# shayekh00/Knowledge_Distillation_for_Sensory_Substitution_in_Multimodal_Models

Hardware: AMD Instinct MI355X
Metric: KD samples/sec/step (7B->0.5B, 336x336) (higher is better)
Workload: dtype bf16; 1 GPU; c1: logit-based KD (LoCa, T=1), 7B->0.5B, 336x336; model=llava-onevision-qwen2-7b (teacher) -> 0.5b (student), global_batch=4, per_gpu_batch=4, seq_len=1536, image=336x336 (2 tiles, 1485 tokens), parallelism=dp1, teacher_lm_stream=bf16

## Files before the change

### knowledge_distillation_for_sensory_substitution_in_multimodal_models_amd/csrc/gemm.hip

```cpp
#include "common.h"

#include <cstring>
#include <type_traits>
#ifdef KD_AB_BUILD
#include <hipblaslt/hipblaslt.h>
#endif

namespace kd {
namespace {

constexpr int BM = 128, BN = 128, BK = 64, NTH = 256;
constexpr int TILE_BYTES = 128 * 64 * 2;
constexpr uint32_t OOB = 0x80000000u;

typedef __attribute__((address_space(3))) void lds_void_t;
typedef __attribute__((address_space(3))) bf16x4 lds_bf16x4_t;

struct GemmP {
    const bf16* A; const bf16* B; void* C;
    const void* bias; const bf16* resid; bf16* aux; const float* alpha_dev;
    int64_t lda, ldb, ldc, ldr, ld_aux;
    int M, N, K;
    float alpha;
    int c_f32, accumulate, bias_f32, act, res_mod;
    int res_f32;
    bf16 *sq, *sk, *sv;
    const float *rcos, *rsin;
    int sS, snq, snkv, shd, shdp;
    int64_t kchunk;
    int64_t split_stride;
    int glu;
    int tile0;
    const float* sa;
    const float* sb;
    int gx, gy;
    float* rst;
    int rst_nt, rst_vs, rst_top2;
    float rst_inv_t;
    int sk_steps, sk_grid;
    float* sk_ws;
    int sk_dp;
    int* sk_cnt;
    int gm;
    int stagger;
    int stag_g;
};

__host__ __device__ inline int sk_wg_of(int64_t s, int64_t tot, int G) { return (int)(((s + 1) * G - 1) / tot); }

__device__ __forceinline__ uint32_t sw_k(int row) { return (uint32_t)((row >> 1) & 7); }
__device__ __forceinline__ uint32_t sw_mn(int k) { return (uint32_t)(((k & 3) | (((k >> 3) & 1) << 2)) << 1); }

__device__ __forceinline__ uint32_t rec_bytes(int64_t rows, int64_t ld) {
    const int64_t b = rows * ld * 2;
    return b <= 0 ? 0u : (b >= 0x7FFFFFFFll ? 0x7FFFFFFFu : (uint32_t)b);
}

__device__ __forceinline__ __amdgpu_buffer_rsrc_t make_rsrc(const void* base, uint32_t bytes) {
    return __builtin_amdgcn_make_buffer_rsrc(const_cast<void*>(base), (short)0, (int)bytes, 0x00020000);
}

__device__ __forceinline__ void dma16(__amdgpu_buffer_rsrc_t rs, char* lds_dst, uint32_t voff) {
    __builtin_amdgcn_raw_ptr_buffer_load_lds(rs, (lds_void_t*)lds_dst, 16, voff, 0, 0, 0);
}

template <bool MN>
__device__ __forceinline__ void stage(char* tile, const bf16* ptr, int64_t ld, int r0, int rows_total,
                                      int k0, int K, int wid, int lane) {
    if (!MN) {
        const int rows_valid = min(128, rows_total - r0);
        auto rs = make_rsrc(ptr + (int64_t)r0 * ld, rec_bytes(rows_valid, ld));
#pragma unroll
        for (int s = 0; s < 4; ++s) {
            const int i = wid * 4 + s;
            const int row = 8 * i + (lane >> 3);
            const int gc = (lane & 7) ^ (int)sw_k(row);
            const int k = k0 + gc * 8;
            const uint32_t voff = (k < K) ? (uint32_t)(((int64_t)row * ld + k) * 2) : OOB;
            dma16(rs, tile + i * 1024, voff);
        }
    } else {
        const int kvalid = max(0, min(64, K - k0));
        auto rs = make_rsrc(ptr + (int64_t)min(k0, K) * ld + r0, rec_bytes(kvalid, ld));
#pragma unroll
        for (int s = 0; s < 4; ++s) {
            const int i = wid * 4 + s;
            const int kr = 4 * i + (lane >> 4);
            const int gc = (lane & 15) ^ (int)sw_mn(kr);
            const int row = r0 + gc * 8;
            const uint32_t voff = (kr < kvalid && row < rows_total) ? (uint32_t)(((int64_t)kr * ld + gc * 8) * 2) : OOB;
            dma16(rs, tile + i * 1024, voff);
        }
    }
}

template <bool MN>
__device__ __forceinline__ bf16x8 frag(const char* tile, int rb, int ks, int lane) {
    if (!MN) {
        const int r = rb + (lane & 15);
        const int kc = ks * 4 + (lane >> 4);
        return *(const bf16x8*)(tile + r * 128 + ((kc ^ (int)sw_k(r)) << 4));
    } else {
        const int g = lane >> 4, q = (lane & 15) >> 2, p = lane & 3;
        const int cc = (rb >> 3) + (p >> 1);
        const int kr0 = ks * 32 + 8 * g + q;
        const int kr1 = kr0 + 4;
        const char* a0 = tile + kr0 * 256 + ((cc ^ (int)sw_mn(kr0)) << 4) + ((p & 1) << 3);
        const char* a1 = tile + kr1 * 256 + ((cc ^ (int)sw_mn(kr1)) << 4) + ((p & 1) << 3);
        bf16x4 h0 = __builtin_amdgcn_ds_read_tr16_b64_v4bf16((lds_bf16x4_t*)a0);
        bf16x4 h1 = __builtin_amdgcn_ds_read_tr16_b64_v4bf16((lds_bf16x4_t*)a1);
        bf16x8 r;
        r[0] = h0[0]; r[1] = h0[1]; r[2] = h0[2]; r[3] = h0[3];
        r[4] = h1[0]; r[5] = h1[1]; r[6] = h1[2]; r[7] = h1[3];
        return r;
    }
}

__device__ __forceinline__ float gelu_tanh(float x) {
    constexpr float c0 = -2.f * 0.7978845608028654f * 1.4426950408889634f;
    constexpr float c1 = c0 * 0.044715f;
    const float e = __builtin_amdgcn_exp2f(x * fmaf(c1, x * x, c0));
    return x * __builtin_amdgcn_rcpf(1.f + e);
}
__device__ __forceinline__ float gelu_erf(float x) { return 0.5f * x * (1.f + erff(x * 0.7071067811865476f)); }
// ... 119 lines not shown
                }
            }
        }
    }
}


constexpr int EPI_G = 8, QKV_G = 2;
constexpr int BK2 = 32, NST = 4, NTH2 = 512;

__device__ __forceinline__ int f4(int row) { return (0x1320 >> (((row >> 2) & 3) * 4)) & 3; }

template <int R, bool MN>
__device__ __forceinline__ void stage2(char* tile, const bf16* ptr, int64_t ld, int r0, int rows_total, int k0, int K,
                                       int wid, int lane, __amdgpu_buffer_rsrc_t rs_k) {
    constexpr int NI = R / 16;
    constexpr int PER = NI / 8;
    if (!MN) {
#pragma unroll
        for (int s = 0; s < PER; ++s) {
            const int i = wid * PER + s;
            const int row = 16 * i + (lane >> 2);
            const int gc = (lane & 3) ^ f4(row);
            const int k = k0 + gc * 8;
            const uint32_t voff = (k < K) ? (uint32_t)(((int64_t)row * ld + k) * 2) : OOB;
            dma16(rs_k, tile + i * 1024, voff);
        }
    } else {
        constexpr int CPR = R / 8;
        constexpr int KPI = 64 / CPR;
        const int kvalid = max(0, min(BK2, K - k0));
        auto rs = make_rsrc(ptr + (int64_t)min(k0, K) * ld + r0, rec_bytes(kvalid, ld));
#pragma unroll
        for (int s = 0; s < PER; ++s) {
            const int i = wid * PER + s;
            const int kr = i * KPI + lane / CPR;
            const int gc = (lane % CPR) ^ (int)sw_mn(kr);
            const int row = r0 + gc * 8;
            const uint32_t voff = (kr < kvalid && row < rows_total) ? (uint32_t)(((int64_t)kr * ld + gc * 8) * 2) : OOB;
            dma16(rs, tile + i * 1024, voff);
        }
    }
}

template <int OFF>
__device__ __forceinline__ bf16x4 ds_read_tr_asm(const char* lds) {
    u32x2 r;
    asm volatile("ds_read_b64_tr_b16 %0, %1 offset:%2" : "=v"(r) : "v"((uint32_t)(uintptr_t)lds), "i"(OFF));
    return __builtin_bit_cast(bf16x4, r);
}

template <int R, bool MN>
__device__ __forceinline__ bf16x8 frag2(const char* tile, int rb, int lane) {
    if (!MN) {
        const int r = rb + (lane & 15);
        const int c = lane >> 4;
        return *(const bf16x8*)(tile + r * 64 + ((c ^ f4(r)) << 4));
    } else {
        constexpr int RB = R * 2;
        const int g = lane >> 4, q = (lane & 15) >> 2, p = lane & 3;
        const int cc = (rb >> 3) + (p >> 1);
        const int kr0 = 8 * g + q;
        const char* a0 = tile + kr0 * RB + ((cc ^ (int)sw_mn(kr0)) << 4) + ((p & 1) << 3);
        const bf16x4 h0 = ds_read_tr_asm<0>(a0);
        const bf16x4 h1 = ds_read_tr_asm<4 * RB>(a0);
        bf16x8 r;
        r[0] = h0[0]; r[1] = h0[1]; r[2] = h0[2]; r[3] = h0[3];
        r[4] = h1[0]; r[5] = h1[1]; r[6] = h1[2]; r[7] = h1[3];
        return r;
    }
}

template <int N> __device__ __forceinline__ void wait_vm() {
    if constexpr (N == 0) asm volatile("s_waitcnt vmcnt(0)" ::: "memory");
    else if constexpr (N == 2) asm volatile("s_waitcnt vmcnt(2)" ::: "memory");
    else if constexpr (N == 3) asm volatile("s_waitcnt vmcnt(3)" ::: "memory");
    else if constexpr (N == 4) asm volatile("s_waitcnt vmcnt(4)" ::: "memory");
    else if constexpr (N == 6) asm volatile("s_waitcnt vmcnt(6)" ::: "memory");
    else if constexpr (N == 8) asm volatile("s_waitcnt vmcnt(8)" ::: "memory");
    else if constexpr (N == 9) asm volatile("s_waitcnt vmcnt(9)" ::: "memory");
    else if constexpr (N == 12) asm volatile("s_waitcnt vmcnt(12)" ::: "memory");
    else if constexpr (N == 15) asm volatile("s_waitcnt vmcnt(15)" ::: "memory");
    else if constexpr (N == 16) asm volatile("s_waitcnt vmcnt(16)" ::: "memory");
    else if constexpr (N == 24) asm volatile("s_waitcnt vmcnt(24)" ::: "memory");
    else static_assert(N == 0, "unsupported vmcnt");
}

template <int BM, int BN, int NS = NST>
constexpr size_t gemm2_lds() {
    constexpr size_t ring = (size_t)NS * (BM + BN) * BK2 * 2;
    constexpr size_t ep16 = (size_t)BM * (BN * 2 + 16);
    constexpr size_t ep32 = (size_t)(BM / 2) * (BN * 4 + 16);
    return ring > ep16 ? (ring > ep32 ? ring : ep32) : (ep16 > ep32 ? ep16 : ep32);
}


__device__ __forceinline__ int acc_row(int lane) { return lane & 15; }
__device__ __forceinline__ int acc_col(int lane) { return (lane >> 4) * 4; }

template <bool L32>
__device__ __forceinline__ int acc_col_of(int j, int lane) {
    return L32 ? (j >> 2) * 32 + 8 * (j & 3) + 4 * (lane >> 5) : j * 16 + acc_col(lane);
}

template <int ACT, int TM, int TN, int MT, int NT, bool F32, bool L32 = false>
__device__ __forceinline__ void epi_to_lds(const f32x4 (&acc)[MT][NT], char* smem, int rs, float alpha,
                                           const f32x4 (&bcol)[NT], int wm, int wn, int lane, int r_lo, int r_hi) {
#pragma unroll
    for (int i = 0; i < MT; ++i) {
        const int lr0 = wm * TM + i * (L32 ? 32 : 16);
        if (lr0 < r_lo || lr0 >= r_hi) continue;
        const int lr = lr0 - r_lo + (L32 ? (lane & 31) : acc_row(lane));
#pragma unroll
        for (int j = 0; j < NT; ++j) {
            const f32x4 a = acc[i][j];
            const int lc = wn * TN + acc_col_of<L32>(j, lane);
            float v[4];
#pragma unroll
            for (int r = 0; r < 4; ++r) v[r] = apply_act(a[r] * alpha + bcol[j][r], ACT);
            if (F32) *(f32x4*)(smem + lr * rs + lc * 4) = (f32x4){v[0], v[1], v[2], v[3]};
            else *(bf16x4*)(smem + lr * rs + lc * 2) = (bf16x4){(bf16)v[0], (bf16)v[1], (bf16)v[2], (bf16)v[3]};
        }
    }
}

template <int TM, int TN, int MT, int NT, bool F32, bool L32 = false>
__device__ __forceinline__ void epi_to_lds_act(int act, const f32x4 (&acc)[MT][NT], char* smem, int rs, float alpha,
                                               const f32x4 (&bcol)[NT], int wm, int wn, int lane, int r_lo, int r_hi) {
    switch (act) {
        case KD_ACT_GELU_TANH: epi_to_lds<KD_ACT_GELU_TANH, TM, TN, MT, NT, F32, L32>(acc, smem, rs, alpha, bcol, wm, wn, lane, r_lo, r_hi); break;
        case KD_ACT_GELU_ERF: epi_to_lds<KD_ACT_GELU_ERF, TM, TN, MT, NT, F32, L32>(acc, smem, rs, alpha, bcol, wm, wn, lane, r_lo, r_hi); break;
        case KD_ACT_SILU: epi_to_lds<KD_ACT_SILU, TM, TN, MT, NT, F32, L32>(acc, smem, rs, alpha, bcol, wm, wn, lane, r_lo, r_hi); break;
        default: epi_to_lds<KD_ACT_NONE, TM, TN, MT, NT, F32, L32>(acc, smem, rs, alpha, bcol, wm, wn, lane, r_lo, r_hi); break;
    }
}

template <int ROWS, int BN, int NTHR, bool F32, bool RES, bool RF, bool ACC>
__device__ __forceinline__ void epi_flush_g(const GemmP& p, const char* smem, int rs, void* dst_, int64_t ld, int m0,
                                            int n0, int tid, bool full) {
    constexpr int EPC = F32 ? 4 : 8;
    constexpr int CPR = BN / EPC;
    static_assert(NTHR % CPR == 0 && (ROWS * CPR) % NTHR == 0, "epi_flush: chunk map");
    constexpr int RSTEP = NTHR / CPR, PER = ROWS * CPR / NTHR, G = PER < EPI_G ? PER : EPI_G;
    static_assert(PER % G == 0, "epi_flush: group");
    using RT = std::conditional_t<RF, f32x4, std::conditional_t<F32, bf16x4, bf16x8>>;
    using VT = std::conditional_t<F32, f32x4, bf16x8>;
    const int c = tid % CPR, lr0 = tid / CPR;
    const int col = n0 + c * EPC;
    if (!full && col >= p.N) return;
#pragma unroll 1
    for (int g0 = 0; g0 < PER; g0 += G) {
        RT rv[G];
        VT cv[G];
        if constexpr (RES || ACC) {
#pragma unroll
            for (int u = 0; u < G; ++u) {
                const int row = full ? m0 + lr0 + (g0 + u) * RSTEP : min(m0 + lr0 + (g0 + u) * RSTEP, p.M - 1);
                if constexpr (RES) {
                    const int64_t rr = p.res_mod > 0 ? row % p.res_mod : row;
                    if constexpr (RF) rv[u] = *(const f32x4*)((const float*)p.resid + rr * p.ldr + col);
                    else rv[u] = *(const RT*)(p.resid + rr * p.ldr + col);
                }
                if constexpr (ACC) {
                    if constexpr (F32) cv[u] = *(const f32x4*)((const float*)dst_ + (int64_t)row * ld + col);
                    else cv[u] = *(const bf16x8*)((const bf16*)dst_ + (int64_t)row * ld + col);
                }
// ... 516 lines not shown
}

template <bool MN>
__device__ __forceinline__ uint32_t voff8(int i, int lane, int64_t ld, int r0, int rows_total) {
    if (!MN) {
        const int row = 16 * i + (lane >> 2);
        const int gc = (lane & 3) ^ f4(row);
        return (uint32_t)((int64_t)row * ld * 2 + gc * 16);
    } else {
        const int kr = 2 * i + (lane >> 5);
        const int gc = (lane & 31) ^ (int)sw_mn(kr);
        return (r0 + gc * 8 < rows_total) ? (uint32_t)((int64_t)kr * ld * 2 + gc * 16) : OOB;
    }
}

struct SkFold {
    float* part; int* cnt;
    int64_t tot, tb;
    int G, wf, piece, np, t;
    int64_t split_base;
};
constexpr int SK_TILE_F32 = 256 * 256;
__device__ __forceinline__ float* sk_slot(const SkFold& f, int w) {
    if (f.tot == 0) return f.part + (f.split_base + w) * SK_TILE_F32;
    const int64_t s0 = f.tot * w / f.G;
    return f.part + ((int64_t)w * 2 + (s0 >= f.tb ? 0 : 1)) * SK_TILE_F32;
}
__device__ __forceinline__ bool sk_fold_tile(const SkFold& f, f32x4 (&acc)[8][8], int tid, int lane, int wid,
                                          char* smem) {
    const int64_t lo = ((int64_t)wid * 64 * 64 + lane) * 4;
    float* mine = sk_slot(f, f.wf + f.piece) + lo;
#pragma unroll
    for (int i = 0; i < 8; ++i)
#pragma unroll
        for (int j = 0; j < 8; ++j) *(f32x4*)(mine + (i * 8 + j) * 256) = acc[i][j];
    asm volatile("s_waitcnt vmcnt(0)" ::: "memory");
    __syncthreads();
    int* flag = (int*)smem;
    if (tid == 0) {
        __builtin_amdgcn_fence(__ATOMIC_RELEASE, "agent");
        asm volatile("s_waitcnt vmcnt(0)" ::: "memory");
        const int old = __hip_atomic_fetch_add(f.cnt + f.t, 1, __ATOMIC_RELAXED, __HIP_MEMORY_SCOPE_AGENT);
        const int last = old == f.np - 1;
        if (last) {
            __builtin_amdgcn_fence(__ATOMIC_ACQUIRE, "agent");
            asm volatile("s_waitcnt vmcnt(0)" ::: "memory");
        }
        flag[0] = last;
    }
    __syncthreads();
    const int last = flag[0];
    __syncthreads();
    if (!last) return false;
#pragma unroll
    for (int h = 0; h < 4; ++h) {
        f32x4 v[16];
        if (f.piece == 0) {
#pragma unroll
            for (int a = 0; a < 16; ++a) v[a] = acc[(h * 16 + a) / 8][(h * 16 + a) % 8];
        } else {
            const float* src = sk_slot(f, f.wf) + lo;
#pragma unroll
            for (int a = 0; a < 16; ++a) v[a] = *(const f32x4*)(src + (h * 16 + a) * 256);
        }
        for (int pc = 1; pc < f.np; ++pc) {
            if (pc == f.piece) {
#pragma unroll
                for (int a = 0; a < 16; ++a) v[a] += acc[(h * 16 + a) / 8][(h * 16 + a) % 8];
            } else {
                const float* src = sk_slot(f, f.wf + pc) + lo;
                f32x4 x[16];
#pragma unroll
                for (int a = 0; a < 16; ++a) x[a] = *(const f32x4*)(src + (h * 16 + a) * 256);
#pragma unroll
                for (int a = 0; a < 16; ++a) v[a] += x[a];
            }
        }
#pragma unroll
        for (int a = 0; a < 16; ++a) acc[(h * 16 + a) / 8][(h * 16 + a) % 8] = v[a];
    }
    return true;
}

template <bool A_MN, bool B_MN, int EXP>
__device__ __forceinline__ void g8_tile(GemmP p, int tm, int tn, char* smem, const SkFold* fold = nullptr) {
    constexpr bool STAMP = EXP & 1, NODMA = EXP & 2, HOT = EXP & 64;
    constexpr bool RS = (EXP & 8) && !A_MN && !B_MN;
    constexpr bool RSTATS = (EXP & 32) && !A_MN && !B_MN;
    constexpr bool TB = (EXP & 256) && !B_MN && !RS;
    const int nkt = (p.K + BK2 - 1) / BK2;

    uint32_t* stamps = nullptr;
    if (STAMP) {
        if ((EXP & 4) && !B_MN) stamps = (uint32_t*)p.sk_ws;
        else { stamps = (uint32_t*)p.aux; p.aux = nullptr; }
    }
    uint64_t mk[2] = {0, 0};
    uint64_t s_pro = 0, s_bar = 0, s_units = 0, s_epi = 0, ts0 = 0;
    uint64_t rt0 = 0;
    if (STAMP) { ts0 = __builtin_amdgcn_s_memtime(); rt0 = __builtin_amdgcn_s_memrealtime(); }
    constexpr int SA = 256 * BK2 * 2, SS = 2 * SA;
    const int tid = threadIdx.x, lane = tid & 63;
    const int wid = __builtin_amdgcn_readfirstlane(tid >> 6);
    const int wm = wid >> 1, wn = wid & 1;
    const int m0 = tm * 256, n0 = tn * 256;
    const int K = p.K;
    const int nk = (K + BK2 - 1) / BK2, nk_full = K / BK2;
    int rot = 0;
    if (p.stagger && nk_full == nk && nk >= 64) {
        const int g = p.stag_g > 0 ? p.stag_g : (p.gm > 0 ? p.gm : GM_GROUP), ngrp = ((p.M + 255) / 256 + g - 1) / g;
        rot = (int)(((int64_t)(tm / g) * nk) / ngrp);
    }
    auto kst = [&](int st) { return (rot == 0 || st >= nk) ? st : (st + rot >= nk ? st + rot - nk : st + rot); };
    const __amdgpu_buffer_rsrc_t rsAk = make_rsrc(p.A + (A_MN ? 0 : (int64_t)m0 * p.lda), A_MN ? 0u : rec_bytes(min(256, p.M - m0), p.lda));
    constexpr bool glu = !B_MN && (EXP & 4);
    const int nb = tn * 128;
    const __amdgpu_buffer_rsrc_t rsBk =
        TB ? make_rsrc(p.B + (int64_t)tn * nkt * (256 * BK2), (uint32_t)nkt * (256 * BK2 * 2))
           : glu ? make_rsrc(p.B, rec_bytes(p.N, p.ldb))
                 : make_rsrc(p.B + (B_MN ? 0 : (int64_t)n0 * p.ldb), B_MN ? 0u : rec_bytes(min(256, p.N - n0), p.ldb));
    uint32_t va[4], vb[4];
#pragma unroll
    for (int u = 0; u < 4; ++u) {
        va[u] = voff8<A_MN>(wid * 4 + u, lane, p.lda, m0, p.M);
        vb[u] = voff8<B_MN>(wid * 4 + u, lane, p.ldb, n0, p.N);
        if (glu && !TB) {
            const int row = 16 * (wid * 4 + u) + (lane >> 2);
            const int gc = (lane & 3) ^ f4(row);
            const int wrow = row < 128 ? nb + row : p.glu + nb + row - 128;
            vb[u] = (uint32_t)((int64_t)wrow * p.ldb * 2 + gc * 16);
        }
        if (TB) vb[u] = (uint32_t)((wid * 4 + u) * 1024 + lane * 16);
    }
    auto dma = [&](int st, int sl, int u, auto full_tag) {
        constexpr bool FULL = decltype(full_tag)::value;
        if (NODMA) return;
        const bool isA = u < 4;
        const bool mn = isA ? A_MN : B_MN;
        const int i = wid * 4 + (u & 3);
        char* dst = smem + sl * SS + (isA ? 0 : SA) + i * 1024;
        uint32_t v = isA ? va[u & 3] : vb[u & 3];
        if (TB && !isA) {
            int soff = kst(st) * (256 * BK2 * 2);
            if (!FULL && st >= nkt) { v = OOB; soff = 0; }
            __builtin_amdgcn_raw_ptr_buffer_load_lds(rsBk, (lds_void_t*)dst, 16, v, soff, 0, 0);
            return;
        }
        if (!mn) {
            int soff = HOT ? 0 : kst(st) * BK2 * 2;
            if (!FULL) {
                const int kleft = K - st * BK2;
                if (kleft < BK2) {
                    const int row = 16 * i + (lane >> 2);
                    const int gc = (lane & 3) ^ f4(row);
                    if (gc * 8 >= kleft) v = OOB;
                    if (kleft <= 0) soff = 0;
                }
            }
            __builtin_amdgcn_raw_ptr_buffer_load_lds(isA ? rsAk : rsBk, (lds_void_t*)dst, 16, v, soff, 0, 0);
        } else {
            const bf16* base = isA ? p.A + m0 : p.B + n0;
            const int64_t ld = isA ? p.lda : p.ldb;
            const int kv = FULL ? BK2 : max(0, min(BK2, K - st * BK2));
            const int ks = kst(st);
            const __amdgpu_buffer_rsrc_t rs = make_rsrc(base + (int64_t)(FULL ? ks * BK2 : min(ks * BK2, K)) * ld, rec_bytes(kv, ld));
            __builtin_amdgcn_raw_ptr_buffer_load_lds(rs, (lds_void_t*)dst, 16, v, 0, 0, 0);
        }
    };
// ... 727 lines not shown
    const dim3 grid(ceil_div(d->M, 256) * ceil_div(d->N, 256));
    p.gx = (int)grid.x; p.gy = 1;
    p.gm = pick_gm(ceil_div(d->M, 256), ceil_div(d->N, 256));
    switch (d->act) {
        case KD_ACT_GELU_TANH: hipLaunchKernelGGL((k_gemm8f8<0, KD_ACT_GELU_TANH>), grid, dim3(NTH8), F8_LDS, st, p); break;
        case KD_ACT_GELU_ERF: hipLaunchKernelGGL((k_gemm8f8<0, KD_ACT_GELU_ERF>), grid, dim3(NTH8), F8_LDS, st, p); break;
        case KD_ACT_SILU: hipLaunchKernelGGL((k_gemm8f8<0, KD_ACT_SILU>), grid, dim3(NTH8), F8_LDS, st, p); break;
        default: hipLaunchKernelGGL((k_gemm8f8<0, KD_ACT_NONE>), grid, dim3(NTH8), F8_LDS, st, p); break;
    }
    KD_LAUNCH_CHECK("k_gemm8f8");
    return KD_OK;
}

int launch_quant_rows_f8(const void* x, int64_t ldx, int R, int K, void* q, int64_t ldq, float* scale, void* stream) {
    KD_CHECK_ARG(x && q && scale, "quant_rows_fp8: null pointer");
    KD_CHECK_SHAPE(R >= 0 && K > 0 && K % 16 == 0 && ldx >= K && ldq >= K && ldx % 8 == 0 && ldq % 8 == 0,
                   "quant_rows_fp8: K % 16 == 0, ldx / ldq >= K and multiples of 8");
    KD_CHECK_ALIGN(x, 16, "quant_rows_fp8: x must be 16-B aligned");
    KD_CHECK_ALIGN(q, 8, "quant_rows_fp8: q must be 8-B aligned");
    if (R == 0) return KD_OK;
    hipLaunchKernelGGL(k_quant_rows_f8, dim3(R), dim3(256), 0, as_stream(stream), (const bf16*)x, ldx, K, (uint8_t*)q, ldq,
                       scale);
    KD_LAUNCH_CHECK("k_quant_rows_f8");
    return KD_OK;
}


__global__ void k_pretile_b(const bf16* __restrict__ W, int64_t ldw, int N, int K, int glu_I, int nkt, int64_t total,
                            bf16* __restrict__ out) {
    for (int64_t idx = (int64_t)blockIdx.x * blockDim.x + threadIdx.x; idx < total; idx += (int64_t)gridDim.x * blockDim.x) {
        const int pc = (int)(idx & 3), r = (int)((idx >> 2) & 255);
        const int64_t ts = idx >> 10;
        const int st = (int)(ts % nkt), t = (int)(ts / nkt);
        const int wrow = glu_I > 0 ? (r < 128 ? 128 * t + r : glu_I + 128 * t + r - 128) : 256 * t + r;
        const int k = st * BK2 + 8 * (pc ^ f4(r));
        bf16x8 v = (bf16x8){};
        if (wrow < N && k < K) v = *(const bf16x8*)(W + (int64_t)wrow * ldw + k);
        *(bf16x8*)(out + idx * 8) = v;
    }
}

size_t gemm_pretile_size(int N, int K, int glu) {
    if (N <= 0 || K <= 0) return 0;
    const int64_t tiles = glu ? (N / 256) : ceil_div(N, 256);
    return (size_t)tiles * ceil_div(K, BK2) * 256 * BK2 * 2;
}

int launch_gemm_pretile(const void* W, int64_t ldw, int N, int K, int glu, void* out, void* stream) {
    KD_CHECK_ARG(W && out, "gemm_pretile: null pointer");
    KD_CHECK_SHAPE(N > 0 && K > 0 && K % 8 == 0 && ldw >= K && ldw % 8 == 0, "gemm_pretile: K % 8 == 0, ldw >= K");
    KD_CHECK_SHAPE(!glu || N % 256 == 0, "gemm_pretile: the SwiGLU layout needs N = 2I with I % 128 == 0");
    KD_CHECK_ALIGN(W, 16, "gemm_pretile: W must be 16-B aligned");
    KD_CHECK_ALIGN(out, 16, "gemm_pretile: out must be 16-B aligned");
    const int nkt = ceil_div(K, BK2);
    const int64_t total = (int64_t)(gemm_pretile_size(N, K, glu) / 16);
    const int grid = (int)std::min<int64_t>((total + 255) / 256, 65536);
    hipLaunchKernelGGL(k_pretile_b, dim3(grid), dim3(256), 0, as_stream(stream), (const bf16*)W, ldw, N, K,
                       glu ? N / 2 : 0, nkt, total, (bf16*)out);
    KD_LAUNCH_CHECK("k_pretile_b");
    return KD_OK;
}

#ifdef KD_AB_BUILD
static bool use_v11(int variant) {
    if (variant == 23) return true;
    if (variant != 0 && variant != 16) return false;
    static const int env = [] { const char* e = std::getenv("KD_GEMM_V11"); return e ? std::atoi(e) : -1; }();
    return env == 1;
}

static bool use_v12(int variant) {
    if (variant == 26) return true;
    if (variant != 0 && variant != 16) return false;
    static const int env = [] { const char* e = std::getenv("KD_GEMM_V12"); return e ? std::atoi(e) : -1; }();
    return env == 1;
}
#endif

static unsigned reduce_grid(int items) {
    const int cap = ab_knob("KD_SK_REDUCE_GRID", 0);
    return (unsigned)(cap > 0 && cap < items ? cap : items);
}

static bool variant_known(int v) {
    if ((v >= 0 && v <= 7) || v == 16 || v == 21 || v == 24 || v == 32) return true;
#ifdef KD_AB_BUILD
    if ((v >= 17 && v <= 20) || v == 22 || v == 23 || (v >= 26 && v <= 28) || v == 30) return true;
#endif
    return false;
}

static bool sk_fits(int64_t tiles, int64_t nk, const kd_gemm_desc* d) {
    const int64_t dp = sk_dp_tiles(tiles, nk);
    return (tiles - dp) * nk >= 2 * SK_GRID && d->workspace && d->workspace_bytes >= sk_workspace_bytes(tiles - dp);
}
static int sk_setup(GemmP& q, int64_t tiles, const kd_gemm_desc* d, hipStream_t st) {
    const int64_t dp = sk_dp_tiles(tiles, ceil_div(d->K, BK2));
    KD_CHECK_ARG(d->workspace && d->workspace_bytes >= sk_workspace_bytes(tiles - dp), "gemm: stream-K workspace too small");
    q.sk_steps = ceil_div(d->K, BK2); q.sk_grid = SK_GRID; q.sk_dp = (int)dp;
    q.sk_cnt = (int*)d->workspace;
    q.sk_ws = (float*)((char*)d->workspace + sk_cnt_bytes(tiles - dp));
    q.gx = (int)dp + SK_GRID; q.gy = 1; q.tile0 = 0;
    if (hipMemsetAsync(q.sk_cnt, 0, sk_cnt_bytes(tiles - dp), st) != hipSuccess)
        return fail(KD_ERR_LAUNCH, "gemm: stream-K ticket memset");
    return KD_OK;
}

int launch_gemm(const kd_gemm_desc* d, void* stream_) {
    KD_CHECK_ARG(d != nullptr, "gemm: null descriptor");
    KD_CHECK_ARG(d->A && d->B && (d->C || d->qkv), "gemm: null operand");
    KD_CHECK_SHAPE(d->M > 0 && d->N > 0 && d->K > 0, "gemm: empty shape");
    KD_CHECK_ARG(d->a_layout == KD_LAYOUT_K_MAJOR || d->a_layout == KD_LAYOUT_MN_MAJOR, "gemm: a_layout");
    KD_CHECK_ARG(d->b_layout == KD_LAYOUT_K_MAJOR || d->b_layout == KD_LAYOUT_MN_MAJOR, "gemm: b_layout");
    KD_CHECK_ARG(d->c_dtype == KD_DTYPE_BF16 || d->c_dtype == KD_DTYPE_F32, "gemm: c_dtype");
    KD_CHECK_ARG(d->ab_dtype == KD_DTYPE_BF16 || d->ab_dtype == KD_DTYPE_FP8_E4M3, "gemm: ab_dtype");
    KD_CHECK_ARG(!d->qkv || d->ab_dtype == KD_DTYPE_BF16, "gemm qkv: bf16 operands only");
    KD_CHECK_ARG(!d->b_pretiled || (d->ab_dtype == KD_DTYPE_BF16 && d->a_layout == KD_LAYOUT_K_MAJOR &&
                                    d->b_layout == KD_LAYOUT_K_MAJOR && !d->row_stats && d->split_k <= 1 &&
                                    (d->variant == 0 || d->variant == 16 || d->variant == 24)),
                 "gemm b_pretiled: K-major bf16 operands on the 256x256 v8 kernel, no split-K / row_stats");
    if (d->ab_dtype == KD_DTYPE_FP8_E4M3) return launch_gemm_f8(d, stream_);
    KD_CHECK_ARG(d->act >= KD_ACT_NONE && d->act <= KD_ACT_DSWIGLU, "gemm: act");
    const bool dact = d->act == KD_ACT_DGELU_TANH || d->act == KD_ACT_DSWIGLU;
    KD_CHECK_ARG(d->act == KD_ACT_NONE || dact || (d->a_layout == KD_LAYOUT_K_MAJOR && d->b_layout == KD_LAYOUT_K_MAJOR &&
                                                   d->c_dtype == KD_DTYPE_BF16),
                 "gemm: an activation epilogue needs K-major operands and a bf16 output");
    if (dact) {
        const int64_t w = d->act == KD_ACT_DSWIGLU ? 2 * (int64_t)d->N : d->N;
        KD_CHECK_ARG(d->aux && d->c_dtype == KD_DTYPE_BF16 && !d->bias && !d->residual && !d->accumulate && d->split_k <= 1 &&
                     d->variant != 1,
                     "gemm backward activation: aux (forward pre-activation), bf16 C, no bias / residual / accumulate / split-K");
        KD_CHECK_SHAPE(d->N % 8 == 0 && d->ldc >= w && d->ld_aux >= w && d->ldc % 8 == 0 && d->ld_aux % 8 == 0 &&
                       (uintptr_t)d->aux % 16 == 0, "gemm backward activation: ldc / ld_aux >= N (2N for dswiglu), 16-B rows");
    }
    KD_CHECK_ARG(variant_known(d->variant),
                 "gemm: unknown variant (the diagnostic / A-B builds 17-20, 22, 23, 26-28 are in the tools' A/B library only)");
    KD_CHECK_ALIGN(d->A, 16, "gemm: A must be 16-B aligned");
    KD_CHECK_ALIGN(d->B, 16, "gemm: B must be 16-B aligned");
    KD_CHECK_ALIGN(d->bias, d->bias_dtype == KD_DTYPE_F32 ? 16 : 8, "gemm: bias must be 16-B (fp32) / 8-B (bf16) aligned");
    KD_CHECK_SHAPE(d->lda % 8 == 0 && d->ldb % 8 == 0, "gemm: lda/ldb must be multiples of 8");
    if (d->a_layout == KD_LAYOUT_K_MAJOR) {
        KD_CHECK_SHAPE(d->K % 8 == 0 && d->lda >= d->K, "gemm: K-major A needs K % 8 == 0, lda >= K");
    } else {
        KD_CHECK_SHAPE(d->M % 8 == 0 && d->lda >= d->M, "gemm: MN-major A needs M % 8 == 0, lda >= M");
        KD_CHECK_SHAPE((uint64_t)64 * d->lda * 2 < 0x7FFFFFFFull, "gemm: lda too large");
    }
    if (d->b_layout == KD_LAYOUT_K_MAJOR) {
        KD_CHECK_SHAPE(d->K % 8 == 0 && d->ldb >= d->K, "gemm: K-major B needs K % 8 == 0, ldb >= K");
    } else {
        KD_CHECK_SHAPE(d->N % 8 == 0 && d->ldb >= d->N, "gemm: MN-major B needs N % 8 == 0, ldb >= N");
    }
    KD_CHECK_SHAPE(d->qkv || d->ldc >= (d->act == KD_ACT_SWIGLU ? d->N / 2 : d->N), "gemm: ldc < N (N/2 for swiglu)");
    KD_CHECK_SHAPE(!d->residual || d->ldr >= d->N, "gemm: ldr < N");
    KD_CHECK_ARG(!d->residual || d->residual_dtype == KD_DTYPE_BF16 ||
                 (d->residual_dtype == KD_DTYPE_F32 && d->c_dtype == KD_DTYPE_F32 && d->act == KD_ACT_NONE),
                 "gemm: an fp32 residual needs an fp32 C and no activation epilogue");
    KD_CHECK_SHAPE(!d->aux || d->ld_aux >= d->N, "gemm: ld_aux < N");
    KD_CHECK_SHAPE((uint64_t)256 * d->lda * 2 < 0x7FFFFFFFull && (uint64_t)256 * d->ldb * 2 < 0x7FFFFFFFull,
                   "gemm: leading dimension too large for 31-bit buffer records");
#ifdef KD_AB_BUILD
    {
        const int bl = ab_knob("KD_GEMM_BLAS", 0);
        if (bl && blas_eligible(d) && (bl == 1 || blas_wins(d))) return blas_gemm(d, as_stream(stream_));
    }
#endif
    GemmP p;
    p.A = (const bf16*)d->A; p.B = (const bf16*)d->B; p.C = d->C;
    p.bias = d->bias; p.resid = (const bf16*)d->residual; p.aux = (bf16*)d->aux; p.alpha_dev = d->alpha_dev;
    p.lda = d->lda; p.ldb = d->ldb; p.ldc = d->ldc; p.ldr = d->ldr; p.ld_aux = d->ld_aux;
    p.M = d->M; p.N = d->N; p.K = d->K; p.alpha = d->alpha;
    p.c_f32 = d->c_dtype == KD_DTYPE_F32; p.accumulate = d->accumulate; p.bias_f32 = d->bias_dtype == KD_DTYPE_F32;
    p.act = d->act;
    p.res_mod = d->residual_row_mod;
    p.res_f32 = d->residual && d->residual_dtype == KD_DTYPE_F32;
    p.sq = p.sk = p.sv = nullptr; p.rcos = p.rsin = nullptr;
    p.sS = p.snq = p.snkv = p.shd = p.shdp = 0;
    if (d->qkv) {
        const kd_qkv_scatter& q = *d->qkv;
        const bool rope = q.cos_t != nullptr;
        KD_CHECK_ARG(q.q && q.k && q.v && (rope == (q.sin_t != nullptr)), "gemm qkv: null q / k / v or cos without sin");
        KD_CHECK_ARG(d->act == KD_ACT_NONE && !d->residual && !d->aux && !d->accumulate && d->c_dtype == KD_DTYPE_BF16 &&
                     d->a_layout == KD_LAYOUT_K_MAJOR && d->b_layout == KD_LAYOUT_K_MAJOR && d->split_k <= 1,
                     "gemm qkv: K-major operands, no activation / residual / aux / accumulate / split-K");
        KD_CHECK_SHAPE(q.S > 0 && d->M % q.S == 0 && q.nq > 0 && q.nkv > 0 && d->N == (q.nq + 2 * q.nkv) * q.hd &&
                       q.hd % 8 == 0 && q.hdp % 8 == 0 && q.hdp >= q.hd && (!rope || (q.hd % 16 == 0 && 128 % q.hd == 0)),
                       "gemm qkv: N = (nq + 2 nkv) hd, M % S == 0, hd / hdp % 8 == 0, RoPE heads dividing 128");
        KD_CHECK_ALIGN(q.q, 16, "gemm qkv: q must be 16-B aligned");
        KD_CHECK_ALIGN(q.k, 16, "gemm qkv: k must be 16-B aligned");
        KD_CHECK_ALIGN(q.v, 16, "gemm qkv: v must be 16-B aligned");
        p.sq = (bf16*)q.q; p.sk = (bf16*)q.k; p.sv = (bf16*)q.v; p.rcos = q.cos_t; p.rsin = q.sin_t;
        p.sS = q.S; p.snq = q.nq; p.snkv = q.nkv; p.shd = q.hd; p.shdp = q.hdp;
    }
    p.kchunk = d->K; p.split_stride = 0; p.glu = 0; p.tile0 = 0;
    p.sa = p.sb = nullptr; p.gx = 0; p.gy = 1;
    p.sk_steps = 0; p.sk_grid = 0; p.sk_ws = nullptr; p.sk_dp = 0; p.sk_cnt = nullptr;
    p.gm = 0;
    p.rst = nullptr; p.rst_nt = p.rst_vs = p.rst_top2 = 0; p.rst_inv_t = 1.f;
    p.stagger = ab_knob("KD_GEMM_STAGGER", 1);
    p.stag_g = 0;
    hipStream_t st = as_stream(stream_);
    const bool amn = d->a_layout == KD_LAYOUT_MN_MAJOR, bmn = d->b_layout == KD_LAYOUT_MN_MAJOR;
    const bool c_ok16 = (d->qkv || ((d->ldc % 8 == 0) && ((uintptr_t)d->C % 16 == 0))) &&
                        (!d->residual || ((d->ldr % 8 == 0) && ((uintptr_t)d->residual % 16 == 0)));
    const bool big_ok = d->N % 8 == 0 && c_ok16 && d->M >= 128 && d->N >= 128 &&
                        ((uint64_t)d->M * d->N >= (1ull << 20) || (d->workspace && d->K >= 2048 && d->split_k != 1)) &&
                        (!amn || d->M % 8 == 0) && (!bmn || d->N % 8 == 0) &&
                        (uint64_t)BK2 * (amn ? d->lda : 0) * 2 < 0x7FFFFFFFull;
    KD_CHECK_ARG(!dact || big_ok, "gemm backward activation: needs the tiled kernels (M, N >= 128, M*N >= 2^20)");
    KD_CHECK_ARG(!d->qkv || (big_ok && d->variant != 1),
                 "gemm qkv: needs the tiled kernels (M, N >= 128, M*N >= 2^20)");
    kd_gemm_desc d1;
    if ((dact || d->qkv) && d->split_k != 1) {
        d1 = *d;
        d1.split_k = 1;
        d = &d1;
    }
    if (d->row_stats) {
        KD_CHECK_ARG(!amn && !bmn && d->c_dtype == KD_DTYPE_BF16 && !d->bias && d->act == KD_ACT_NONE && !d->residual &&
                         !d->aux && !d->accumulate && !d->qkv && d->ab_dtype == KD_DTYPE_BF16,
                     "gemm row_stats: K-major bf16 operands, bf16 C, no bias / act / residual / aux / accumulate");
        KD_CHECK_SHAPE(d->N % 8 == 0 && (d->row_stats_vs <= 0 || d->row_stats_vs % 8 == 0) && big_ok,
                       "gemm row_stats: N and row_stats_vs multiples of 8, the tiled kernels' shapes");
        KD_CHECK_ARG(d->row_stats_inv_t > 0.f, "gemm row_stats: row_stats_inv_t must be > 0");
        KD_CHECK_ALIGN(d->row_stats, 16, "gemm row_stats: 16-B aligned");
        GemmP pk = p;
        pk.rst = d->row_stats; pk.rst_nt = ceil_div(d->N, 256); pk.rst_vs = d->row_stats_vs;
        pk.rst_inv_t = d->row_stats_inv_t; pk.rst_top2 = d->row_stats_top2 ? 1 : 0;
        pk.gm = pick_gm(ceil_div(d->M, 256), ceil_div(d->N, 256));
        const dim3 grid(ceil_div(d->M, 256) * ceil_div(d->N, 256), 1);
        pk.gx = (int)grid.x; pk.gy = 1; pk.tile0 = 0;
        hipLaunchKernelGGL((k_gemm8<false, false, 32>), grid, dim3(NTH8), (gemm2_lds<256, 256>()), st, pk);
        KD_LAUNCH_CHECK("k_gemm8 (row stats)");
        return KD_OK;
    }
    if (d->act == KD_ACT_SWIGLU) {
        KD_CHECK_SHAPE(d->N % 256 == 0 && d->M >= 1, "gemm swiglu: N = 2I needs I % 128 == 0");
        KD_CHECK_ARG(!d->bias && !d->residual && !d->accumulate && d->split_k <= 1,
                     "gemm swiglu: no bias / residual / accumulate / split-K");
        KD_CHECK_ARG(!amn && !bmn && d->c_dtype == KD_DTYPE_BF16 && c_ok16 && d->ldc >= d->N / 2,
                     "gemm swiglu: K-major operands, 16-B aligned bf16 output [M, N/2]");
        KD_CHECK_ARG(!d->aux || (d->ld_aux % 8 == 0 && (uintptr_t)d->aux % 16 == 0), "gemm swiglu: aux alignment");
        GemmP pk = p;
        pk.glu = d->N / 2; pk.act = KD_ACT_NONE;
        pk.gm = pick_gm(ceil_div(d->M, 256), d->N / 256);
        const dim3 grid(ceil_div(d->M, 256) * (d->N / 256), 1);
        pk.gx = (int)grid.x; pk.gy = 1;
#ifdef KD_AB_BUILD
        if (d->variant == 20) hipLaunchKernelGGL((k_gemm9<false, false>), grid, dim3(NTH9), (gemm2_lds<256, 256>()), st, pk);
        else if (!d->b_pretiled && use_v11(d->variant)) hipLaunchKernelGGL((k_gemm11<4>), grid, dim3(NTH8), (gemm2_lds<256, 256>()), st, pk);
        else if (d->variant == 27) hipLaunchKernelGGL((k_gemm12<4 | 256>), grid, dim3(NTH8), (gemm2_lds<256, 256>()), st, pk);
        else if (!d->b_pretiled && use_v12(d->variant)) hipLaunchKernelGGL((k_gemm12<4>), grid, dim3(NTH8), (gemm2_lds<256, 256>()), st, pk);
        else if (d->variant == 22)
            hipLaunchKernelGGL((k_gemm8<false, false, 12>), grid, dim3(NTH8), (gemm2_lds<256, 256>()), st, pk);
        else if (d->variant == 28) {
            KD_CHECK_ARG(d->workspace && d->workspace_bytes >= (uint64_t)grid.x * (4 * 8 + 4) * 4, "gemm swiglu stamps: workspace");
            pk.sk_ws = (float*)d->workspace;
            hipLaunchKernelGGL((k_gemm8<false, false, 5>), grid, dim3(NTH8), (gemm2_lds<256, 256>()), st, pk);
        }
        else if (glu_epi_v0()) hipLaunchKernelGGL((k_gemm8<false, false, 4 | 512>), grid, dim3(NTH8), (gemm2_lds<256, 256>()), st, pk);
        else
#endif
        if (d->b_pretiled) hipLaunchKernelGGL((k_gemm8<false, false, 4 | 256>), grid, dim3(NTH8), (gemm2_lds<256, 256>()), st, pk);
        else if (d->variant == 21 && sk_fits(grid.x, ceil_div(d->K, BK2), d)) {
            if (const int rc = sk_setup(pk, grid.x, d, st); rc != KD_OK) return rc;
            hipLaunchKernelGGL((k_gemm8<false, false, 4 | 1024>), dim3(pk.gx), dim3(NTH8), (gemm2_lds<256, 256>()), st, pk);
        }
        else hipLaunchKernelGGL((k_gemm8<false, false, 4>), grid, dim3(NTH8), (gemm2_lds<256, 256>()), st, pk);
        KD_LAUNCH_CHECK("k_gemm<swiglu>");
        return KD_OK;
    }
    if (d->b_pretiled) {
        KD_CHECK_ARG(d->N % 8 == 0 && c_ok16, "gemm b_pretiled: N % 8 == 0 and 16-B aligned C / residual rows");
        GemmP q = p;
        q.gm = pick_gm(ceil_div(d->M, 256), ceil_div(d->N, 256));
        const dim3 grid(ceil_div(d->M, 256) * ceil_div(d->N, 256), 1);
        q.gx = (int)grid.x; q.gy = 1; q.tile0 = 0;
        hipLaunchKernelGGL((k_gemm8<false, false, 256>), grid, dim3(NTH8), (gemm2_lds<256, 256>()), st, q);
        KD_LAUNCH_CHECK("k_gemm8 (b_pretiled)");
        return KD_OK;
    }
#ifdef KD_AB_BUILD
    if (d->variant == 30) {
        KD_CHECK_ARG(!amn && !bmn && (!d->qkv || !d->qkv->cos_t || 128 % d->qkv->hd == 0) && !d->row_stats &&
                     !d->b_pretiled && !dact && d->act != KD_ACT_SWIGLU && d->split_k <= 1 && d->N % 8 == 0 && c_ok16,
                     "gemm variant 30 (v8n): K-major A and B, no SwiGLU / backward activation / row statistics / split, "
                     "N % 8 == 0; a RoPE q|k|v scatter needs 128 % head_dim == 0");
        GemmP q = p;
        q.gm = pick_gm(ceil_div(d->M, 256), ceil_div(d->N, 128));
// ... 108 lines not shown
            const size_t cnt_b = sk_cnt_bytes(nt);
            KD_CHECK_ARG(d->workspace_bytes >= cnt_b + (size_t)nt * pl.split * SK_TILE_F32 * 4,
                         "gemm: split-K fold workspace too small");
            GemmP q = p;
            q.kchunk = pl.kchunk; q.tile0 = pl.dp_tiles; q.gx = nt; q.gy = pl.split;
            q.sk_cnt = (int*)d->workspace; q.sk_ws = (float*)((char*)d->workspace + cnt_b);
            if (hipMemsetAsync(q.sk_cnt, 0, cnt_b, st) != hipSuccess) return fail(KD_ERR_LAUNCH, "gemm: split-K ticket memset");
            const dim3 grid((unsigned)nt, (unsigned)pl.split);
            const size_t lds = gemm2_lds<256, 256>();
            if (!amn && !bmn) hipLaunchKernelGGL((k_gemm8<false, false, 2048>), grid, dim3(NTH8), lds, st, q);
            else if (!amn && bmn) hipLaunchKernelGGL((k_gemm8<false, true, 2048>), grid, dim3(NTH8), lds, st, q);
            else if (amn && bmn) hipLaunchKernelGGL((k_gemm8<true, true, 2048>), grid, dim3(NTH8), lds, st, q);
            else hipLaunchKernelGGL((k_gemm8<true, false, 2048>), grid, dim3(NTH8), lds, st, q);
            KD_LAUNCH_CHECK("k_gemm8 (split-K fold)");
            return KD_OK;
        }
        GemmP pk = p;
        pk.C = d->workspace; pk.ldc = d->N; pk.c_f32 = 1; pk.accumulate = 0; pk.alpha = 1.f;
        pk.alpha_dev = nullptr; pk.bias = nullptr; pk.aux = nullptr; pk.resid = nullptr; pk.act = KD_ACT_NONE;
        pk.kchunk = pl.kchunk; pk.split_stride = (int64_t)d->M * d->N; pk.tile0 = pl.dp_tiles;
        launch_tiles(pk, tiles - pl.dp_tiles, (unsigned)pl.split);
        KD_LAUNCH_CHECK("k_gemm (split tiles)");
        p.split_stride = (int64_t)d->M * d->N;
        p.tile0 = pl.dp_tiles;
        p.gx = tiles - pl.dp_tiles; p.gy = tbm * tbn / 1024;
        hipLaunchKernelGGL(k_splitk_reduce, dim3(reduce_grid(p.gx * p.gy)), dim3(256), 0, st,
                           (const float*)d->workspace, pl.split, p, tbm, tbn);
        KD_LAUNCH_CHECK("k_splitk_reduce");
        return KD_OK;
    }
    const int tiles = ceil_div(d->M, BM) * ceil_div(d->N, BN);
    const size_t smem = 4 * TILE_BYTES;
    p.gx = tiles; p.gy = 1;
    if (!amn && !bmn) hipLaunchKernelGGL((k_gemm<false, false>), dim3(tiles), dim3(NTH), smem, st, p);
    else if (!amn && bmn) hipLaunchKernelGGL((k_gemm<false, true>), dim3(tiles), dim3(NTH), smem, st, p);
    else if (amn && bmn) hipLaunchKernelGGL((k_gemm<true, true>), dim3(tiles), dim3(NTH), smem, st, p);
    else hipLaunchKernelGGL((k_gemm<true, false>), dim3(tiles), dim3(NTH), smem, st, p);
    KD_LAUNCH_CHECK("k_gemm");
    return KD_OK;
}

bool gemm_group_member_ok(const kd_gemm_desc* d) {
    return d && d->A && d->B && d->C && d->M >= 128 && d->N >= 128 && d->K > 0 &&
           d->a_layout == KD_LAYOUT_MN_MAJOR && d->b_layout == KD_LAYOUT_MN_MAJOR && d->ab_dtype == KD_DTYPE_BF16 &&
           d->c_dtype == KD_DTYPE_F32 && !d->bias && d->act == KD_ACT_NONE && !d->residual && !d->aux && !d->qkv &&
           !d->row_stats && !d->alpha_dev && !d->b_pretiled && d->M % 8 == 0 && d->N % 8 == 0 && d->lda % 8 == 0 &&
           d->ldb % 8 == 0 && d->ldc % 8 == 0 && d->lda >= d->M && d->ldb >= d->N && d->ldc >= d->N &&
           (uintptr_t)d->A % 16 == 0 && (uintptr_t)d->B % 16 == 0 && (uintptr_t)d->C % 16 == 0 &&
           (uint64_t)256 * d->lda * 2 < 0x7FFFFFFFull && (uint64_t)256 * d->ldb * 2 < 0x7FFFFFFFull;
}

int launch_gemm_group(const kd_gemm_desc* const* ds, int n, void* stream_) {
    KD_CHECK_ARG(ds != nullptr, "gemm group: null member list");
    KD_CHECK_ARG(n >= 1 && n <= GROUP_MAX, "gemm group: 1 to 4 members");
    GemmGroupP g;
    std::memset(&g, 0, sizeof(g));
    int total = 0;
    for (int i = 0; i < n; ++i) {
        const kd_gemm_desc* d = ds[i];
        KD_CHECK_ARG(d != nullptr, "gemm group: null member");
        KD_CHECK_ARG(d->A && d->B && d->C, "gemm group: null operand");
        KD_CHECK_ARG(d->M > 0 && d->N > 0 && d->K > 0, "gemm group: empty shape");
        KD_CHECK_ARG(d->a_layout == KD_LAYOUT_MN_MAJOR && d->b_layout == KD_LAYOUT_MN_MAJOR,
                     "gemm group: MN-major A and B only (weight gradients)");
        KD_CHECK_ARG(d->ab_dtype == KD_DTYPE_BF16 && d->c_dtype == KD_DTYPE_F32, "gemm group: bf16 operands, fp32 C");
        KD_CHECK_ARG(!d->bias && d->act == KD_ACT_NONE && !d->residual && !d->aux && !d->qkv && !d->row_stats &&
                     !d->alpha_dev && !d->b_pretiled,
                     "gemm group: no bias / activation / residual / aux / scatter / row statistics / device alpha");
        KD_CHECK_ARG(d->M % 8 == 0 && d->N % 8 == 0, "gemm group: M % 8 == 0 and N % 8 == 0");
        KD_CHECK_ARG(d->M >= 128 && d->N >= 128, "gemm group: M, N >= 128 (the 256 x 256 tile kernel)");
        KD_CHECK_ARG(d->lda % 8 == 0 && d->ldb % 8 == 0 && d->ldc % 8 == 0 && d->lda >= d->M && d->ldb >= d->N &&
                     d->ldc >= d->N, "gemm group: lda >= M, ldb >= N, ldc >= N, multiples of 8");
        KD_CHECK_ARG((uintptr_t)d->A % 16 == 0 && (uintptr_t)d->B % 16 == 0 && (uintptr_t)d->C % 16 == 0,
                     "gemm group: A, B and C must be 16-B aligned");
        KD_CHECK_ARG((uint64_t)256 * d->lda * 2 < 0x7FFFFFFFull && (uint64_t)256 * d->ldb * 2 < 0x7FFFFFFFull,
                     "gemm group: leading dimension too large for 31-bit buffer records");
        GemmP& p = g.p[i];
        p.A = (const bf16*)d->A; p.B = (const bf16*)d->B; p.C = d->C;
        p.lda = d->lda; p.ldb = d->ldb; p.ldc = d->ldc;
        p.M = d->M; p.N = d->N; p.K = d->K; p.alpha = d->alpha;
        p.c_f32 = 1; p.accumulate = d->accumulate;
        p.kchunk = d->K; p.gy = 1; p.rst_inv_t = 1.f;
        p.stagger = ab_knob("KD_GEMM_STAGGER", 1);
        const int tiles_m = ceil_div(d->M, 256), tiles_n = ceil_div(d->N, 256);
        p.gm = pick_gm(tiles_m, tiles_n);
        p.gx = tiles_m * tiles_n;
        g.t0[i] = total;
        total += p.gx;
    }
    for (int i = n; i < GROUP_MAX; ++i) g.t0[i] = total;
    hipLaunchKernelGGL(k_gemm8_group, dim3((unsigned)total), dim3(NTH8), (gemm2_lds<256, 256>()), as_stream(stream_), g);
    KD_LAUNCH_CHECK("k_gemm8_group");
    return KD_OK;
}

int gemm_plan_query(const kd_gemm_desc* d, int32_t* var, int32_t* split, int32_t* dp) {
    KD_CHECK_ARG(d && var && split && dp, "gemm_plan: null pointer");
    KD_CHECK_SHAPE(d->M > 0 && d->N > 0 && d->K > 0, "gemm_plan: empty shape");
    const bool amn = d->a_layout == KD_LAYOUT_MN_MAJOR, bmn = d->b_layout == KD_LAYOUT_MN_MAJOR;
    const bool big_ok = d->N % 8 == 0 && d->M >= 128 && d->N >= 128 &&
                        ((uint64_t)d->M * d->N >= (1ull << 20) || (d->workspace && d->K >= 2048 && d->split_k != 1)) &&
                        (!amn || d->M % 8 == 0) && (!bmn || d->N % 8 == 0);
    if (d->act == KD_ACT_SWIGLU) { *var = 16; *split = 1; *dp = 0; return KD_OK; }
#ifdef KD_AB_BUILD
    if (d->variant == 30) { *var = 30; *split = 1; *dp = 0; return KD_OK; }
#endif
    if (d->variant == 1 || !big_ok) { *var = 1; *split = 1; *dp = 0; return KD_OK; }
    const GemmPlan pl = plan_gemm(d, d->workspace ? d->workspace_bytes : 0);
    *var = pl.var; *split = pl.split; *dp = pl.dp_tiles;
    return KD_OK;
}

size_t gemm_workspace_size(const kd_gemm_desc* d) {
    if (!d || d->M <= 0 || d->N <= 0 || d->K <= 0 || d->variant == 1 || d->act == KD_ACT_SWIGLU) return 0;
    const GemmPlan pl = plan_gemm(d, ~0ull);
    if (pl.var == 21) return sk_workspace_bytes((int64_t)ceil_div(d->M, 256) * ceil_div(d->N, 256) - pl.dp_tiles);
    return pl.split > 1 ? (size_t)pl.split * d->M * d->N * 4 : 0;
}

}
```

Before: 29.83 samples/s.

## Use half-width 256x128 tiles for ragged edge tiles in MN-major GEMMs

Adds a tail-tile kernel path that runs a 256x128 (or 128x256) tile when the remaining N (or M) extent of an edge tile is at most 128, for GEMMs whose B operand is MN-major. This avoids spending MFMA work and DMA bandwidth on the padded half of a 256x256 tile. The tail path reuses the same pipelined ring, stagger rotation and epilogue, with its own fragment loads and vmcnt wait count. Default is on, and an env knob or variant 33 switches back to wide tails. Variants 33 and 34 also let small shapes use the tiled kernel.

```diff
diff --git a/knowledge_distillation_for_sensory_substitution_in_multimodal_models_amd/csrc/gemm.hip b/knowledge_distillation_for_sensory_substitution_in_multimodal_models_amd/csrc/gemm.hip
--- a/knowledge_distillation_for_sensory_substitution_in_multimodal_models_amd/csrc/gemm.hip
+++ b/knowledge_distillation_for_sensory_substitution_in_multimodal_models_amd/csrc/gemm.hip
@@ -40,6 +40,7 @@
     int sk_steps, sk_grid;
     float* sk_ws;
     int sk_dp;
+    int wide_tails;
     int* sk_cnt;
     int gm;
     int stagger;
@@ -325,6 +326,7 @@
     else if constexpr (N == 12) asm volatile("s_waitcnt vmcnt(12)" ::: "memory");
     else if constexpr (N == 15) asm volatile("s_waitcnt vmcnt(15)" ::: "memory");
     else if constexpr (N == 16) asm volatile("s_waitcnt vmcnt(16)" ::: "memory");
+    else if constexpr (N == 18) asm volatile("s_waitcnt vmcnt(18)" ::: "memory");
     else if constexpr (N == 24) asm volatile("s_waitcnt vmcnt(24)" ::: "memory");
     else static_assert(N == 0, "unsupported vmcnt");
 }
@@ -1007,8 +1009,152 @@
     return true;
 }
 
+template <int R>
+__device__ __forceinline__ uint32_t voff8_mn(int i, int lane, int64_t ld, int r0, int rows_total) {
+    constexpr int CPR = R / 8, KPI = 64 / CPR;
+    const int kr = KPI * i + lane / CPR;
+    const int gc = (lane % CPR) ^ (int)sw_mn(kr);
+    return (r0 + gc * 8 < rows_total) ? (uint32_t)((int64_t)kr * ld * 2 + gc * 16) : OOB;
+}
+
+template <bool A_MN, bool B_MN, bool NN>
+__device__ __forceinline__ void g8_tile_tail(const GemmP& p, int tm, int tn, char* smem) {
+    static_assert(NN ? B_MN : A_MN, "g8_tile_tail: the halved operand is MN-major");
+    constexpr int RA = NN ? 256 : 128, RB = NN ? 128 : 256;
+    constexpr int MT = RA / 32, NT = RB / 32;
+    constexpr int DA = RA / 64, DB = RB / 64, ND = DA + DB;
+    constexpr int SA = 256 * BK2 * 2, SS = 2 * SA;
+    const int tid = threadIdx.x, lane = tid & 63;
+    const int wid = __builtin_amdgcn_readfirstlane(tid >> 6);
+    const int wm = wid >> 1, wn = wid & 1;
+    const int m0 = tm * 256, n0 = tn * 256;
+    const int K = p.K;
+    const int nk = (K + BK2 - 1) / BK2, nk_full = K / BK2;
+    int rot = 0;
+    if (p.stagger && nk_full == nk && nk >= 64) {
+        const int g = p.stag_g > 0 ? p.stag_g : (p.gm > 0 ? p.gm : GM_GROUP), ngrp = ((p.M + 255) / 256 + g - 1) / g;
+        rot = (int)(((int64_t)(tm / g) * nk) / ngrp);
+    }
+    auto kst = [&](int st) { return (rot == 0 || st >= nk) ? st : (st + rot >= nk ? st + rot - nk : st + rot); };
+    const __amdgpu_buffer_rsrc_t rsAk = make_rsrc(p.A + (A_MN ? 0 : (int64_t)m0 * p.lda), A_MN ? 0u : rec_bytes(min(256, p.M - m0), p.lda));
+    uint32_t va[DA], vb[DB];
+#pragma unroll
+    for (int u = 0; u < DA; ++u) {
+        if constexpr (A_MN) va[u] = voff8_mn<RA>(wid * DA + u, lane, p.lda, m0, p.M);
+        else va[u] = voff8<false>(wid * DA + u, lane, p.lda, m0, p.M);
+    }
+#pragma unroll
+    for (int u = 0; u < DB; ++u) vb[u] = voff8_mn<RB>(wid * DB + u, lane, p.ldb, n0, p.N);
+    auto dma = [&](int st, int sl, int u, auto full_tag) {
+        constexpr bool FULL = decltype(full_tag)::value;
+        const bool isA = u < DA;
+        const int w = isA ? u : u - DA;
+        const int i = wid * (isA ? DA : DB) + w;
+        char* dst = smem + sl * SS + (isA ? 0 : SA) + i * 1024;
+        uint32_t v = isA ? va[isA ? w : 0] : vb[isA ? 0 : w];
+        if (isA && !A_MN) {
+            int soff = kst(st) * BK2 * 2;
+            if (!FULL) {
+                const int kleft = K - st * BK2;
+                if (kleft < BK2) {
+                    const int row = 16 * i + (lane >> 2);
+                    const int gc = (lane & 3) ^ f4(row);
+                    if (gc * 8 >= kleft) v = OOB;
+                    if (kleft <= 0) soff = 0;
+                }
+            }
+            __builtin_amdgcn_raw_ptr_buffer_load_lds(rsAk, (lds_void_t*)dst, 16, v, soff, 0, 0);
+        } else {
+            const bf16* base = isA ? p.A + m0 : p.B + n0;
+            const int64_t ld = isA ? p.lda : p.ldb;
+            const int kv = FULL ? BK2 : max(0, min(BK2, K - st * BK2));
+            const int ks = kst(st);
+            const __amdgpu_buffer_rsrc_t rs = make_rsrc(base + (int64_t)(FULL ? ks * BK2 : min(ks * BK2, K)) * ld, rec_bytes(kv, ld));
+            __builtin_amdgcn_raw_ptr_buffer_load_lds(rs, (lds_void_t*)dst, 16, v, 0, 0, 0);
+        }
+    };
+    using FullT = std::integral_constant<bool, true>;
+    using PartT = std::integral_constant<bool, false>;
+    f32x4 acc[MT][NT];
+#pragma unroll
+    for (int i = 0; i < MT; ++i)
+#pragma unroll
+        for (int j = 0; j < NT; ++j) acc[i][j] = (f32x4){0.f, 0.f, 0.f, 0.f};
+    const int ra = wm * (RA / 2), cb = wn * (RB / 2);
+#pragma unroll
+    for (int st = 0; st < NS8; ++st)
+#pragma unroll
+        for (int u = 0; u < ND; ++u) dma(st, st, u, PartT{});
+    wait_vm<3 * ND>();
+    __builtin_amdgcn_s_barrier();
+    bf16x8 xa[MT], xb[NT], ya[MT], yb[NT];
+#pragma unroll
+    for (int u = 0; u < MT; ++u) xa[u] = frag2<RA, A_MN>(smem, ra + u * 16, lane);
+#pragma unroll
+    for (int u = 0; u < NT; ++u) xb[u] = frag2<RB, B_MN>(smem + SA, cb + u * 16, lane);
+#define KD_G8T_SYNC()                                                                                        \
+    {                                                                                                         \
+        asm volatile("s_waitcnt lgkmcnt(0)" ::: "memory");                                                    \
+        wait_vm<2 * ND>();                                                                                    \
+        __builtin_amdgcn_s_barrier();                                                                         \
+    }
+    KD_G8T_SYNC()
+    __builtin_amdgcn_sched_barrier(0);
+#define KD_SB __builtin_amdgcn_sched_barrier(0);
+#define KD_G8T_STEP(SL, CA, CB, NA, NB, FT)                                                                  \
+    {                                                                                                         \
+        const int t_ = t + (SL);                                                                              \
+        const char* na_ = smem + (((SL) + 1) % NS8) * SS;                                                     \
+        _Pragma("unroll") for (int q = 0; q < MT * NT; ++q) {                                                 \
+            if (q == MT * NT - 1) {                                                                           \
+                KD_G8T_SYNC()                                                                                 \
+                KD_SB                                                                                         \
+                mfma_agpr_last(acc[q / NT][q % NT], CB[q % NT], CA[q / NT], t_ + 1 == nk);                    \
+            } else mfma_agpr(acc[q / NT][q % NT], CB[q % NT], CA[q / NT]);                                    \
+            KD_SB                                                                                             \
+            if (q % 4 == 0 && q / 4 < ND) dma(t_ + NS8, (SL), q / 4, FT{});                                   \
+            if (q % 2 == 1 && q / 2 < MT) NA[q / 2 < MT ? q / 2 : 0] = frag2<RA, A_MN>(na_, ra + (q / 2) * 16, lane); \
+            if (q % 2 == 1 && q / 2 >= MT && q / 2 < MT + NT)                                                 \
+                NB[q / 2 >= MT && q / 2 < MT + NT ? q / 2 - MT : 0] = frag2<RB, B_MN>(na_ + SA, cb + (q / 2 - MT) * 16, lane); \
+            KD_SB                                                                                             \
+        }                                                                                                     \
+    }
+    int t = 0;
+    for (; t + 2 * NS8 <= nk_full; t += NS8) {
+        KD_G8T_STEP(0, xa, xb, ya, yb, FullT)
+        KD_G8T_STEP(1, ya, yb, xa, xb, FullT)
+        KD_G8T_STEP(2, xa, xb, ya, yb, FullT)
+        KD_G8T_STEP(3, ya, yb, xa, xb, FullT)
+    }
+    for (; t + NS8 <= nk; t += NS8) {
+        KD_G8T_STEP(0, xa, xb, ya, yb, PartT)
+        KD_G8T_STEP(1, ya, yb, xa, xb, PartT)
+        KD_G8T_STEP(2, xa, xb, ya, yb, PartT)
+        KD_G8T_STEP(3, ya, yb, xa, xb, PartT)
+    }
+    const int rem = nk - t;
+    if (rem > 0) KD_G8T_STEP(0, xa, xb, ya, yb, PartT)
+    if (rem > 1) KD_G8T_STEP(1, ya, yb, xa, xb, PartT)
+    if (rem > 2) KD_G8T_STEP(2, xa, xb, ya, yb, PartT)
+#undef KD_G8T_STEP
+#undef KD_G8T_SYNC
+#undef KD_SB
+    asm volatile("s_waitcnt vmcnt(0) lgkmcnt(0)\n\ts_nop 15\n\ts_nop 15" ::: "memory");
+    __builtin_amdgcn_sched_barrier(0);
+    __syncthreads();
+    epilogue2<RA, RB, 2, 2, RA / 2, RB / 2, MT, NT, NTH8, false>(p, acc, smem, m0, n0, wm, wn, lane, tid);
+}
+
 template <bool A_MN, bool B_MN, int EXP>
 __device__ __forceinline__ void g8_tile(GemmP p, int tm, int tn, char* smem, const SkFold* fold = nullptr) {
+    if constexpr (EXP == 0 && B_MN) {
+        if (!p.wide_tails) {
+            if (p.N - tn * 256 <= 128) { g8_tile_tail<A_MN, B_MN, true>(p, tm, tn, smem); return; }
+            if constexpr (A_MN) {
+                if (p.M - tm * 256 <= 128) { g8_tile_tail<A_MN, B_MN, false>(p, tm, tn, smem); return; }
+            }
+        }
+    }
     constexpr bool STAMP = EXP & 1, NODMA = EXP & 2, HOT = EXP & 64;
     constexpr bool RS = (EXP & 8) && !A_MN && !B_MN;
     constexpr bool RSTATS = (EXP & 32) && !A_MN && !B_MN;
@@ -1902,8 +2048,12 @@
     return (unsigned)(cap > 0 && cap < items ? cap : items);
 }
 
+static bool v8_any_size(int v) { return v == 33 || v == 34; }
+
+static bool tail_tiles_off() { return ab_knob("KD_GEMM_TAIL_TILES", 1) == 0; }
+
 static bool variant_known(int v) {
-    if ((v >= 0 && v <= 7) || v == 16 || v == 21 || v == 24 || v == 32) return true;
+    if ((v >= 0 && v <= 7) || v == 16 || v == 21 || v == 24 || v == 32 || v == 33 || v == 34) return true;
 #ifdef KD_AB_BUILD
     if ((v >= 17 && v <= 20) || v == 22 || v == 23 || (v >= 26 && v <= 28) || v == 30) return true;
 #endif
@@ -2018,12 +2168,14 @@
     p.rst = nullptr; p.rst_nt = p.rst_vs = p.rst_top2 = 0; p.rst_inv_t = 1.f;
     p.stagger = ab_knob("KD_GEMM_STAGGER", 1);
     p.stag_g = 0;
+    p.wide_tails = d->variant == 33 || tail_tiles_off();
     hipStream_t st = as_stream(stream_);
     const bool amn = d->a_layout == KD_LAYOUT_MN_MAJOR, bmn = d->b_layout == KD_LAYOUT_MN_MAJOR;
     const bool c_ok16 = (d->qkv || ((d->ldc % 8 == 0) && ((uintptr_t)d->C % 16 == 0))) &&
                         (!d->residual || ((d->ldr % 8 == 0) && ((uintptr_t)d->residual % 16 == 0)));
     const bool big_ok = d->N % 8 == 0 && c_ok16 && d->M >= 128 && d->N >= 128 &&
-                        ((uint64_t)d->M * d->N >= (1ull << 20) || (d->workspace && d->K >= 2048 && d->split_k != 1)) &&
+                        ((uint64_t)d->M * d->N >= (1ull << 20) || (d->workspace && d->K >= 2048 && d->split_k != 1) ||
+                         v8_any_size(d->variant)) &&
                         (!amn || d->M % 8 == 0) && (!bmn || d->N % 8 == 0) &&
                         (uint64_t)BK2 * (amn ? d->lda : 0) * 2 < 0x7FFFFFFFull;
     KD_CHECK_ARG(!dact || big_ok, "gemm backward activation: needs the tiled kernels (M, N >= 128, M*N >= 2^20)");
@@ -2298,6 +2450,7 @@
         p.c_f32 = 1; p.accumulate = d->accumulate;
         p.kchunk = d->K; p.gy = 1; p.rst_inv_t = 1.f;
         p.stagger = ab_knob("KD_GEMM_STAGGER", 1);
+        p.wide_tails = tail_tiles_off();
         const int tiles_m = ceil_div(d->M, 256), tiles_n = ceil_div(d->N, 256);
         p.gm = pick_gm(tiles_m, tiles_n);
         p.gx = tiles_m * tiles_n;
@@ -2315,7 +2468,8 @@
     KD_CHECK_SHAPE(d->M > 0 && d->N > 0 && d->K > 0, "gemm_plan: empty shape");
     const bool amn = d->a_layout == KD_LAYOUT_MN_MAJOR, bmn = d->b_layout == KD_LAYOUT_MN_MAJOR;
     const bool big_ok = d->N % 8 == 0 && d->M >= 128 && d->N >= 128 &&
-                        ((uint64_t)d->M * d->N >= (1ull << 20) || (d->workspace && d->K >= 2048 && d->split_k != 1)) &&
+                        ((uint64_t)d->M * d->N >= (1ull << 20) || (d->workspace && d->K >= 2048 && d->split_k != 1) ||
+                         v8_any_size(d->variant)) &&
                         (!amn || d->M % 8 == 0) && (!bmn || d->N % 8 == 0);
     if (d->act == KD_ACT_SWIGLU) { *var = 16; *split = 1; *dp = 0; return KD_OK; }
 #ifdef KD_AB_BUILD
```

Result: no change. 29.93 samples/s, median of 4 (+0.3%).
